# apache/arrow

Measured on AMD Instinct MI355X. Metric: filter_take_mrows_per_s, higher is better.
Workload: dtype int64; 1 GPU; Filter+Take int64[1000000000] + validity (10% null), boolean mask 10% true, FilterOptions::DROP; take indices = the mask's row numbers (monotonic; indices_nonzero: uint64 through CallFunction, GetTakeIndices: uint32 in the mirror), no boundscheck; inputs = splitmix64 streams of SURVEY.md 8(d) (seeds 1,2,3); rows=1000000000, selected_rows=99992053, parallelism=single-gpu

## Files before the change

### arrow_amd/_lib.py

```python
from __future__ import annotations

import ctypes as C
import os

_HERE = os.path.dirname(os.path.abspath(__file__))
LIB_PATH = os.path.join(_HERE, "libarrow_amd.so")

ARX_OK = 0
ARX_OUT_OF_MEMORY = -1
ARX_INVALID = -4
ARX_CAPACITY_ERROR = -6
ARX_INDEX_ERROR = -7
ARX_NOT_IMPLEMENTED = -10
ARX_DEVICE_ERROR = -100

ABI_VERSION = 5

FILTER_DROP, FILTER_EMIT_NULL = 0, 1
SORT_ASCENDING, SORT_DESCENDING = 0, 1
NULLS_AT_START, NULLS_AT_END = 0, 1


class ArrowAmdError(Exception):
    """Base class; subclasses mirror pyarrow.lib.ArrowInvalid & friends."""
# ... 61 lines not shown
        ("validity", C.c_void_p),
        ("offsets", C.c_void_p),
        ("data", C.c_void_p),
        ("offset", C.c_int64),
        ("length", C.c_int64),
        ("null_count", C.c_int64),
    ]


_p, _i64, _int, _u64, _u32, _sz = C.c_void_p, C.c_int64, C.c_int, C.c_uint64, C.c_uint32, C.c_size_t
_span = C.POINTER(ArxSpan)
_bspan = C.POINTER(ArxBinarySpan)

SIGNATURES = {
    "arx_last_error": (C.c_char_p, []),
    "arx_abi_version": (_int, []),
    "arx_device_count": (_int, []),
    "arx_set_option": (_int, [C.c_char_p, _i64]),
    "arx_get_option": (_int, [C.c_char_p, C.POINTER(_i64)]),
    "arx_get_counter": (_i64, [C.c_char_p]),
    "arx_filter_workspace_bytes": (_sz, [_i64]),
    "arx_filter_count": (_int, [_span, _int, _p, _sz, C.POINTER(_i64), _p]),
    "arx_filter_count_async": (_int, [_span, _int, _p, _sz, _p]),
    "arx_filter_count_nulls": (_int, [_span, _span, _int, _p, _sz, C.POINTER(_i64), C.POINTER(_i64), _p]),
    "arx_filter_exec": (_int, [_span, _int, _span, _int, _p, _i64, _p, _p, _p]),
    "arx_mask_to_indices": (_int, [_span, _int, _p, _i64, _int, _p, _p, _p]),
    "arx_filter_compact_form": (_int, [_int, _int, _int, _int, _i64, _i64]),
    "arx_take_workspace_bytes": (_sz, []),
    "arx_check_index_bounds": (_int, [_span, _int, _u64, _p, _sz, _p]),
    "arx_take": (_int, [_span, _int, _span, _int, _p, _p, _p, _p]),
    "arx_take_rows": (_int, [_span, _i64, _span, _int, _p, _p, _p, _p]),
    "arx_take_bits": (_int, [_span, _span, _int, _p, _p, _p, _p]),
    "arx_binary_take_workspace_bytes": (_sz, [_i64]),
    "arx_binary_take_offsets": (_int, [_bspan, _span, _int, _p, _sz, _p, _p, _p, C.POINTER(_i64), _p]),
    "arx_binary_take_data": (_int, [_bspan, _i64, _p, _sz, _p, _i64, _p, _p]),
    "arx_large_binary_take_workspace_bytes": (_sz, [_i64]),
    "arx_large_binary_take_offsets": (_int, [_bspan, _span, _int, _p, _sz, _p, _p, _p, C.POINTER(_i64), _p]),
    "arx_large_binary_take_data": (_int, [_bspan, _i64, _p, _sz, _p, _i64, _p, _p]),
    "arx_list_take_data": (_int, [_bspan, _int, _i64, _p, _sz, _p, _i64, _p, _p]),
    "arx_large_list_take_data": (_int, [_bspan, _int, _i64, _p, _sz, _p, _i64, _p, _p]),
    "arx_plain_byte_array_offsets": (_int, [_p, _sz, _i64, C.c_int32, _p]),
    "arx_rle_scan_runs": (_int, [_p, _sz, _int, _i64, _u32, _u64, _p, _i64, C.POINTER(_i64), C.POINTER(_i64)]),
    "arx_rle_decode_u32": (_int, [_p, _sz, _p, _i64, _int, _i64, _p, _p]),
    "arx_rle_decode_equals_bitmap": (_int, [_p, _sz, _p, _i64, _int, _i64, _u32, _p, _p]),
    "arx_expand_by_mask": (_int, [_p, _int, _span, _p, _p, _p]),
    "arx_rle_levels_to_bitmap": (_int, [_p, _p, _i64, _p, _p, _p, _p]),
    "arx_rle_scan_runs_equals": (_int, [_p, _sz, _int, _i64, _u32, _u32, _u64, _p, _i64, C.POINTER(_i64), C.POINTER(_i64)]),
    "arx_levels_to_list_workspace_bytes": (_sz, [_i64]),
# ... 203 lines not shown
```

### arrow_amd/csrc/plugin/common.inc

```

std::atomic<int64_t> g_gpu_calls{0};
std::atomic<int64_t> g_stock_calls{0};
std::atomic<int64_t> g_min_rows{1 << 16};
std::atomic<int64_t> g_min_rows_streaming{INT64_MAX};
std::atomic<int64_t> g_filter_morsel_rows{[] {
  const char* env = std::getenv("ARROW_AMD_FILTER_MORSEL_ROWS");
  return env != nullptr ? static_cast<int64_t>(std::strtoll(env, nullptr, 10)) : int64_t(1) << 20;
}()};

std::atomic<bool> g_parquet_pinned_staging{true};
std::atomic<bool> g_parquet_device_levels{true};
std::atomic<int> g_parquet_read_threads{4};
std::atomic<int64_t> g_parquet_read_part_bytes{int64_t(1) << 23};
std::atomic<bool> g_parquet_device_snappy{[] {
  const char* env = std::getenv("ARROW_AMD_PARQUET_DEVICE_SNAPPY");
  return env == nullptr || std::strtoll(env, nullptr, 10) != 0;
}()};
std::atomic<int64_t> g_parquet_device_snappy_pages{0};
std::atomic<bool> g_parquet_device_gzip{true};
std::atomic<int64_t> g_parquet_device_gzip_pages{0};
std::atomic<int64_t> g_parquet_copied_pages{0};

std::atomic<int64_t> g_aggregate_flush_rows{[] {
  const char* env = std::getenv("ARROW_AMD_AGGREGATE_FLUSH_ROWS");
// ... 68 lines not shown
    case ARX_CAPACITY_ERROR: return Status::CapacityError(msg);
    case ARX_INDEX_ERROR: return Status::IndexError(msg);
    case ARX_NOT_IMPLEMENTED: return Status::NotImplemented(msg);
    case ARX_OUT_OF_MEMORY: return Status::OutOfMemory(msg);
    default: return Status::UnknownError(msg);
  }
}

#define HIP_RETURN_NOT_OK(call)                                                        \
  do {                                                                                 \
    hipError_t e__ = (call);                                                           \
    if (e__ != hipSuccess)                                                             \
      return Status::IOError("HIP: ", hipGetErrorString(e__), " in " #call);           \
  } while (0)

thread_local hipStream_t t_stream = nullptr;

class DeviceScratch {
 public:
  ~DeviceScratch() {
    for (auto& s : slots_) {
      if (s.ptr) (void)hipFree(s.ptr);
    }
  }
  hipStream_t PeekStream() const { return stream_; }
  Status Stream(hipStream_t* out) {
    if (!stream_) {
      HIP_RETURN_NOT_OK(hipStreamCreateWithFlags(&stream_, hipStreamNonBlocking));
      t_stream = stream_;
    }
    *out = stream_;
    return Status::OK();
  }
  Status Get(int slot, size_t bytes, void** out) {
    if (slots_.size() <= static_cast<size_t>(slot)) slots_.resize(slot + 1);
    Slot& s = slots_[slot];
    bytes = (bytes + 255) & ~size_t(255);
    if (s.size < bytes) {
      if (s.ptr) HIP_RETURN_NOT_OK(hipFree(s.ptr));
      s.ptr = nullptr;
      s.size = 0;
      const size_t want = std::max<size_t>(bytes + bytes / 4, 1 << 20);
      HIP_RETURN_NOT_OK(hipMalloc(&s.ptr, want));
      s.size = want;
    }
    *out = s.ptr;
    return Status::OK();
  }

 private:
  struct Slot { void* ptr = nullptr; size_t size = 0; };
  std::vector<Slot> slots_;
  hipStream_t stream_ = nullptr;
};
thread_local DeviceScratch t_scratch;

class PinnedStaging {
 public:
  ~PinnedStaging() {
    if (ptr_) (void)hipHostFree(ptr_);
  }
  Status Reserve(size_t bytes, uint8_t** out) {
    if (size_ < bytes) {
      if (ptr_) HIP_RETURN_NOT_OK(hipHostFree(ptr_));
      ptr_ = nullptr;
      size_ = 0;
      const size_t want = std::max<size_t>(bytes + bytes / 4, size_t(1) << 20);
      HIP_RETURN_NOT_OK(hipHostMalloc(&ptr_, want, hipHostMallocDefault));
      size_ = want;
    }
    *out = static_cast<uint8_t*>(ptr_);
    return Status::OK();
  }
  void Trim(size_t keep_at_most) {
    if (size_ > keep_at_most && ptr_ != nullptr) {
      (void)hipHostFree(ptr_);
      ptr_ = nullptr;
      size_ = 0;
// ... 106 lines not shown
```

### arrow_amd/csrc/plugin/selection.inc

```
StockKernel g_stock_filter;

arrow::Result<std::unique_ptr<cp::KernelState>> FilterInit(cp::KernelContext* ctx,
                                                           const cp::KernelInitArgs& args) {
  auto state = std::make_unique<ShimState<cp::FilterOptions>>();
  if (g_stock_filter.init) {
    ARROW_ASSIGN_OR_RAISE(state->stock, g_stock_filter.init(ctx, args));
  }
  if (args.options != nullptr) {
    state->options = *static_cast<const cp::FilterOptions*>(args.options);
  }
  return state;
}

Status BooleanTakeOnDevice(const ArxSpan& dv, const ArxSpan& di, int tid, hipStream_t st, ArrayData* out_arr) {
  const int64_t m = di.length;
  const int64_t bytes = ((m + 63) / 64) * 8;
  const bool allocate_validity = dv.null_count != 0 || di.null_count != 0;
  out_arr->length = m;
  out_arr->buffers.resize(2);
  out_arr->buffers[0] = nullptr;
  ARROW_ASSIGN_OR_RAISE(out_arr->buffers[1], AllocDevice(bytes));
  void* d_valid = nullptr;
  void* d_counter = nullptr;
  if (allocate_validity) {
// ... 106 lines not shown
      if (allocate_validity) {
        ARROW_ASSIGN_OR_RAISE(out_arr->buffers[0], AllocDevice(((n + 63) / 64) * 8));
        d_valid = reinterpret_cast<void*>(out_arr->buffers[0]->mutable_address());
      }
      ARROW_RETURN_NOT_OK(FromArx(arx_filter_exec(&dv, w, &dm, null_sel, ws, n,
                                                  reinterpret_cast<void*>(out_arr->buffers[1]->mutable_address()),
                                                  d_valid, st)));
      int64_t selected = 0, set_bits = 0;
      HIP_RETURN_NOT_OK(hipMemcpyAsync(&selected, ws, 8, hipMemcpyDeviceToHost, st));
      if (allocate_validity) {
        void* cws = nullptr;
        ARROW_RETURN_NOT_OK(t_scratch.Get(kCounter, 64, &cws));
        ARROW_RETURN_NOT_OK(FromArx(arx_bitmap_popcount(d_valid, 0, n, cws, 64, &set_bits, st)));
      } else {
        HIP_RETURN_NOT_OK(hipStreamSynchronize(st));
      }
      out_arr->length = selected;
      out_arr->null_count = allocate_validity ? selected - set_bits : 0;
      static_cast<RocmBuffer*>(out_arr->buffers[1].get())->Shrink(selected * w);
      if (allocate_validity) static_cast<RocmBuffer*>(out_arr->buffers[0].get())->Shrink(((selected + 63) / 64) * 8);
      CountGpu(kFnFilter);
      return Status::OK();
    }
    int64_t out_len = 0, out_nulls = 0;
    if (allocate_validity) {
      ARROW_RETURN_NOT_OK(FromArx(arx_filter_count_nulls(&dv, &dm, null_sel, ws, ws_bytes, &out_len, &out_nulls, st)));
    } else {
      ARROW_RETURN_NOT_OK(FromArx(arx_filter_count(&dm, null_sel, ws, ws_bytes, &out_len, st)));
    }
    out_arr->length = out_len;
    out_arr->buffers.resize(2);
    ARROW_ASSIGN_OR_RAISE(out_arr->buffers[1], AllocDevice(out_len * w));
    out_arr->buffers[0] = nullptr;
    void* d_valid = nullptr;
    if (allocate_validity) {
      ARROW_ASSIGN_OR_RAISE(out_arr->buffers[0], AllocDevice(((out_len + 63) / 64) * 8));
      d_valid = reinterpret_cast<void*>(out_arr->buffers[0]->mutable_address());
    }
    ARROW_RETURN_NOT_OK(FromArx(arx_filter_exec(&dv, w, &dm, null_sel, ws, out_len,
                                                reinterpret_cast<void*>(out_arr->buffers[1]->mutable_address()),
                                                d_valid, st)));
    out_arr->null_count = allocate_validity ? out_nulls : 0;
    HIP_RETURN_NOT_OK(hipStreamSynchronize(st));
    CountGpu(kFnFilter);
    return Status::OK();
  }
  if (w == 0 || filter.type->id() != Type::BOOL || values.length < g_min_rows.load() ||
      !IsHost(values) || !IsHost(filter)) {
    return RunStock(kFnFilter, g_stock_filter, state->stock.get(), ctx, batch, out);
  }
  hipStream_t st;
  ARROW_RETURN_NOT_OK(t_scratch.Stream(&st));
  ArxSpan dv{}, dm{};
  ARROW_RETURN_NOT_OK(Upload(values, w, kValues, kValidity, st, &dv));
  ARROW_RETURN_NOT_OK(Upload(filter, 0, kArg2, kArg2Validity, st, &dm));
  const size_t ws_bytes = arx_filter_workspace_bytes(filter.length);
  void* ws = nullptr;
  ARROW_RETURN_NOT_OK(t_scratch.Get(kWs, ws_bytes, &ws));
  int64_t out_len = 0;
  ARROW_RETURN_NOT_OK(FromArx(arx_filter_count(&dm, null_sel, ws, ws_bytes, &out_len, st)));

  ArrayData* out_arr = out->array_data().get();
  const bool filter_null_count_is_zero = filter.null_count == 0;
  if (values.null_count == 0 && (null_sel == ARX_FILTER_DROP || filter_null_count_is_zero)) {
    out_arr->null_count = 0;
  } else {
// ... 326 lines not shown
```

### arrow_amd/csrc/plugin/vector_hash.inc

```
enum HashVectorKind { kHashUnique = 0, kHashValueCounts, kHashDictEncode };

struct DeviceHashState : public cp::KernelState {
  HashVectorKind kind = kHashUnique;
  std::unique_ptr<cp::KernelState> stock;
  bool used_stock = false, used_device = false;
  bool encode_nulls = false;
  std::shared_ptr<arrow::DataType> type;
  int width = 0;
  std::shared_ptr<Buffer> table_buf, counts_buf;
  void* table = nullptr;
  int64_t max_groups = 0, num_groups = 0, counts_cap = 0;
};

StockKernel g_stock_unique, g_stock_value_counts, g_stock_dict_encode;
cp::VectorKernel::FinalizeFunc g_stock_unique_finalize = nullptr, g_stock_value_counts_finalize = nullptr,
                               g_stock_dict_encode_finalize = nullptr;

template <HashVectorKind KIND>
const StockKernel& StockHashKernel() {
  return KIND == kHashUnique ? g_stock_unique : KIND == kHashValueCounts ? g_stock_value_counts : g_stock_dict_encode;
}

Status HashUniques(DeviceHashState* s, hipStream_t st, std::shared_ptr<Buffer>* values, std::shared_ptr<Buffer>* validity,
                   int64_t* null_count) {
// ... 293 lines not shown
  } else {
    const int num = NonZeroNumericTypeId(in.type->id());
    if (num < 0) return Status::NotImplemented("arrow_amd: indices_nonzero of device-resident ", in.type->ToString(), " arrays");
    static const int widths[10] = {1, 1, 2, 2, 4, 4, 8, 8, 4, 8};
    ARROW_ASSIGN_OR_RAISE(bits, AllocDevice(((n + 63) / 64) * 8 + 8));
    const uint64_t zero = 0;
    const uint8_t* base = static_cast<const uint8_t*>(dv.data) + dv.offset * widths[num];
    if (n > 0) {
      ARROW_RETURN_NOT_OK(FromArx(arx_compare_numeric(ARX_CMP_NOT_EQUAL, num, base, nullptr, nullptr, &zero, n,
                                                      reinterpret_cast<uint64_t*>(bits->mutable_address()), st)));
    }
    dm.data = reinterpret_cast<const void*>(bits->address());
    dm.offset = 0;
    if (dm.validity != nullptr && dv.offset != 0) {
      ARROW_ASSIGN_OR_RAISE(rebased, AllocDevice(((n + 63) / 64) * 8 + 8));
      ARROW_RETURN_NOT_OK(FromArx(arx_bitmap_copy(dv.validity, dv.offset, n, reinterpret_cast<void*>(rebased->mutable_address()), st)));
      dm.validity = reinterpret_cast<const void*>(rebased->address());
    }
  }
  const size_t ws_bytes = arx_filter_workspace_bytes(n);
  void* ws = nullptr;
  ARROW_RETURN_NOT_OK(t_scratch.Get(kWs, ws_bytes, &ws));
  int64_t cnt = 0;
  if (n > 0) ARROW_RETURN_NOT_OK(FromArx(arx_filter_count(&dm, ARX_FILTER_DROP, ws, ws_bytes, &cnt, st)));
  void* d_idx = nullptr;
  ARROW_RETURN_NOT_OK(t_scratch.Get(kArg2, static_cast<size_t>(cnt) * 4 + 64, &d_idx));
  ARROW_ASSIGN_OR_RAISE(auto out_values, AllocDevice(std::max<int64_t>(cnt, 1) * 8));
  bool direct = false;
  if (cnt > 0) {
    direct = arx_mask_to_indices(&dm, ARX_FILTER_DROP, ws, cnt, 8, reinterpret_cast<void*>(out_values->mutable_address()), nullptr, st) == ARX_OK;
  }
  if (cnt > 0 && !direct) {
    ARROW_RETURN_NOT_OK(FromArx(arx_mask_to_indices(&dm, ARX_FILTER_DROP, ws, cnt, 4, d_idx, nullptr, st)));
    ArxSpan di{nullptr, d_idx, 0, cnt, 0};
    void* flag = nullptr;
    ARROW_RETURN_NOT_OK(t_scratch.Get(kFlag, 64, &flag));
    ARROW_RETURN_NOT_OK(FromArx(arx_cast_numeric(&di, ARX_NUM_UINT32, ARX_NUM_UINT64, 1, 1, flag, 64,
                                                 reinterpret_cast<void*>(out_values->mutable_address()), st)));
  }
  HIP_RETURN_NOT_OK(hipStreamSynchronize(st));
  CountGpu(kFnFilter);
  out->value = ArrayData::Make(arrow::uint64(), cnt, {nullptr, std::move(out_values)}, 0);
  return Status::OK();
}

Status RegisterIndicesNonZero(cp::FunctionRegistry* reg) {
  ARROW_ASSIGN_OR_RAISE(auto fn, reg->GetFunction("indices_nonzero"));
// ... 72 lines not shown
```

### arrow_amd/csrc/selection.hip

```cpp
#include "arx_common.h"

#include <string.h>

#include <algorithm>
#include <type_traits>

namespace arx {

struct FilterWsHeader {
  int64_t total;
  int64_t ntiles;
  int64_t ngroups;
  int64_t length;
  int64_t valid;
  int64_t pad[3];
};
static_assert(sizeof(FilterWsHeader) == 64, "header is one 64-byte line");

struct FilterWsView {
  FilterWsHeader* hdr;
  int64_t* group_excl;
  int64_t* group_total;
  uint32_t* tile_counts;
  int64_t* group_valid;
};

static inline int64_t num_tiles(int64_t length) { return ceil_div(length, kTileRows); }
static inline int64_t num_groups(int64_t length) {
  return ceil_div(num_tiles(length), kTilesPerGroup);
}

static inline FilterWsView ws_view(void* ws, int64_t length) {
  FilterWsView v;
  const int64_t ng = num_groups(length);
  uint8_t* p = static_cast<uint8_t*>(ws);
  v.hdr = reinterpret_cast<FilterWsHeader*>(p);
  v.group_excl = reinterpret_cast<int64_t*>(p + 64);
  v.group_total = v.group_excl + ng;
  v.tile_counts = reinterpret_cast<uint32_t*>(v.group_total + ng);
  v.group_valid = reinterpret_cast<int64_t*>(v.tile_counts + ng * kTilesPerGroup);
  return v;
}

__device__ __forceinline__ uint64_t emit_word(const Bits& mask, const Bits& mvalid, int64_t w,
                                              bool emit_null, bool invert,
                                              uint64_t* mask_valid_out) {
  uint64_t m = load_word(mask, w);
  const uint64_t mv = load_word(mvalid, w);
  *mask_valid_out = mv;
  if (emit_null || invert) {
    const uint64_t in_range = load_word(Bits{nullptr, 0, mask.length, 0}, w);
    if (invert) m = ~m & in_range;
    if (emit_null) return (m | ~mv) & in_range;
  }
  return m & mv;
}

template <bool VALID>
__global__ __launch_bounds__(kBlock) void count_kernel(Bits mask, Bits mvalid, Bits vvalid, int emit_null,
                                                       int invert, int64_t ntiles,
                                                       uint32_t* tile_counts,
                                                       int64_t* group_total, int64_t* group_valid) {
  __shared__ uint32_t wave_sums[kWavesPerBlock];
  __shared__ uint32_t wave_valid[kWavesPerBlock];
  const int lane = lane_id();
  const int wave = threadIdx.x >> 6;
  const int64_t group = blockIdx.x;
  const int64_t t0 = group * kTilesPerGroup + wave * 16;
  uint32_t mine = 0;
  uint32_t kv = 0;
#pragma unroll 4
  for (int i = 0; i < 16; ++i) {
    const int64_t t = t0 + i;
    uint32_t k = 0;
    if (t < ntiles) {
      uint64_t mv;
      const uint64_t e = emit_word(mask, mvalid, t * 64 + lane, emit_null != 0, invert != 0, &mv);
      k = __popcll(e);
      if constexpr (VALID) kv += __popcll(e & mv & load_word(vvalid, t * 64 + lane));
    }
    const uint32_t s = wave_reduce_sum_u32(k);
    if (lane == i) mine = s;
  }
  if (lane < 16) tile_counts[t0 + lane] = mine;
  const uint32_t wsum = wave_reduce_sum_u32(lane < 16 ? mine : 0u);
  if (lane == 0) wave_sums[wave] = wsum;
  if constexpr (VALID) {
    const uint32_t vsum = wave_reduce_sum_u32(kv);
    if (lane == 0) wave_valid[wave] = vsum;
  }
  __syncthreads();
  if (threadIdx.x == 0) {
    int64_t s = 0, v = 0;
    for (int i = 0; i < kWavesPerBlock; ++i) {
      s += wave_sums[i];
      if constexpr (VALID) v += wave_valid[i];
    }
    group_total[group] = s;
    if constexpr (VALID) group_valid[group] = v;
  }
}

__global__ __launch_bounds__(1024) void scan_kernel(const int64_t* group_total, int64_t ngroups,
                                                    int64_t* group_excl, FilterWsHeader* hdr,
                                                    const int64_t* group_valid = nullptr) {
  __shared__ int64_t wave_tot[16];
  __shared__ int64_t carry_s;
  __shared__ unsigned long long valid_s;
  const int tid = threadIdx.x;
  const int lane = tid & 63;
  const int wave = tid >> 6;
  if (tid == 0) carry_s = 0;
  if (tid == 0) valid_s = 0;
  __syncthreads();
  if (group_valid != nullptr) {
    int64_t mine = 0;
    for (int64_t i = tid; i < ngroups; i += 1024) mine += group_valid[i];
#pragma unroll
    for (int d = 32; d >= 1; d >>= 1) mine += __shfl_xor(mine, d, 64);
    if (lane == 0 && mine != 0) atomicAdd(&valid_s, static_cast<unsigned long long>(mine));
    __syncthreads();
  }
  for (int64_t base = 0; base < ngroups; base += 1024) {
    const int64_t i = base + tid;
    const int64_t v = i < ngroups ? group_total[i] : 0;
    int64_t x = v;
#pragma unroll
    for (int d = 1; d < 64; d <<= 1) {
      const int64_t n = __shfl_up(x, d, 64);
      if (lane >= d) x += n;
    }
    if (lane == 63) wave_tot[wave] = x;
    __syncthreads();
    int64_t wave_prefix = 0;
    for (int k = 0; k < wave; ++k) wave_prefix += wave_tot[k];
    const int64_t carry = carry_s;
    if (i < ngroups) group_excl[i] = carry + wave_prefix + x - v;
    __syncthreads();
    if (tid == 1023) carry_s = carry + wave_prefix + x;
    __syncthreads();
  }
  if (tid == 0) {
    hdr->total = carry_s;
    hdr->valid = static_cast<int64_t>(valid_s);
  }
}

struct CompactArgs {
  const uint8_t* values;
  Bits mask;
  Bits mvalid;
  Bits vvalid;
  int64_t length;
  int64_t ntiles;
  const uint32_t* tile_counts;
  const int64_t* group_excl;
  uint8_t* out_data;
  uint64_t* out_validity;
  int emit_null;
  int invert;
  int values_aligned16;
};

constexpr int kFlushBytes = 2048;

template <int RING>
struct __attribute__((aligned(16))) CompactLds {
  uint8_t ring[kWavesPerBlock][RING];
  uint64_t vbits[kWavesPerBlock][72];
};

template <int W>
struct ElemT;
template <> struct ElemT<1> { using type = uint8_t; };
template <> struct ElemT<2> { using type = uint16_t; };
template <> struct ElemT<4> { using type = uint32_t; };
template <> struct ElemT<8> { using type = uint64_t; };
template <> struct ElemT<16> { using type = uint4; };
struct Elem32 { uint4 lo, hi; };
template <> struct ElemT<32> { using type = Elem32; };

template <int W>
__device__ __forceinline__ typename ElemT<W>::type zero_elem() {
  if constexpr (W == 32) {
// ... 387 lines not shown
  const uint32_t p = incl - k;
  const int total = static_cast<int>(__shfl(incl, 63, 64));
  if (total == 0) return;

  const int64_t grp = t >> 6;
  const int tin = static_cast<int>(t & 63);
  const uint32_t cprev = lane < tin ? a.tile_counts[grp * kTilesPerGroup + lane] : 0u;
  const int64_t off = a.group_excl[grp] + wave_reduce_sum_u32(cprev);

  uint16_t* sel = lds.sel[wave];
  const bool want_validity = a.out_validity != nullptr;
  if (want_validity) lds.vs[wave][lane] = load_word(a.vvalid, w) & mv;
  if constexpr (EMIT) lds.zw[wave][lane] = Ew & ~mv;

  const E* __restrict__ values = IOTA ? nullptr : reinterpret_cast<const E*>(a.values) + t * kTileRows;
  E* __restrict__ out = reinterpret_cast<E*>(a.out_data);
  const int head = static_cast<int>(off & 63);
  const int nsteps = (head + total + 63) >> 6;
  const int64_t word0 = off >> 6;
  constexpr int kStepsPerWindow = kSparseWindow / 64;

  uint64_t m = Ew;
  uint32_t rk = p;
  for (int step0 = 0; step0 < nsteps; step0 += kStepsPerWindow) {
    const int win_lo = step0 * 64 - head;
    const int win_hi = win_lo + kSparseWindow;
    while (m != 0 && static_cast<int>(rk) < win_hi) {
      const int bpos = __ffsll(static_cast<unsigned long long>(m)) - 1;
      m &= m - 1;
      sel[static_cast<int>(rk) - win_lo] = static_cast<uint16_t>(lane * 64 + bpos);
      ++rk;
    }
    wave_lds_sync();
    const int step_end = (step0 + kStepsPerWindow) < nsteps ? (step0 + kStepsPerWindow) : nsteps;
    const int first_listed = win_lo < 0 ? 0 : win_lo;
    for (int i0 = step0; i0 < step_end; i0 += U) {
      int s[U];
      bool act[U];
      int r[U];
      E v[U];
#pragma unroll
      for (int u = 0; u < U; ++u) {
        s[u] = (i0 + u) * 64 + lane - head;
        act[u] = s[u] >= 0 && s[u] < total && (i0 + u) < step_end;
        r[u] = sel[(act[u] ? s[u] : first_listed) - win_lo];
      }
#pragma unroll
      for (int u = 0; u < U; ++u) {
        if constexpr (IOTA) {
          if constexpr (W <= 8) v[u] = static_cast<E>(t * kTileRows + r[u]);
        } else {
          v[u] = sel_load<W>(values + r[u], (kSelNt & 1) != 0);
        }
      }
#pragma unroll
      for (int u = 0; u < U; ++u) {
        if ((i0 + u) >= step_end) break;
        E e = v[u];
        if constexpr (EMIT) {
          if ((lds.zw[wave][r[u] >> 6] >> (r[u] & 63)) & 1ull) e = zero_elem<W>();
        }
        if (act[u]) sel_store<W>(out + off + s[u], e);
        if (want_validity) {
          const bool vbit = act[u] && ((lds.vs[wave][r[u] >> 6] >> (r[u] & 63)) & 1ull);
          const uint64_t bal = __ballot(vbit);
          const uint64_t owned = __ballot(act[u]);
          if (lane == 0) {
            uint64_t* dst = a.out_validity + word0 + i0 + u;
            if (owned == ~uint64_t(0)) {
              *dst = bal;
            } else if (bal != 0) {
              atomicOr(reinterpret_cast<unsigned long long*>(dst), static_cast<unsigned long long>(bal));
            }
          }
        }
      }
    }
    wave_lds_sync();
  }
}

template <int W>
__global__ __launch_bounds__(kBlock) void expand_kernel(CompactArgs a) {
  using E = typename ElemT<W>::type;
  __shared__ uint64_t words[kWavesPerBlock][64];
  __shared__ uint32_t before[kWavesPerBlock][64];
  const int lane = lane_id();
  const int wave = __builtin_amdgcn_readfirstlane(threadIdx.x >> 6);
  const int64_t t = static_cast<int64_t>(blockIdx.x) * kWavesPerBlock + wave;
  if (t >= a.ntiles) return;
  uint64_t mv;
  const uint64_t mw = emit_word(a.mask, a.mvalid, t * 64 + lane, false, false, &mv);
  const uint32_t k = __popcll(mw);
  const uint32_t incl = wave_inclusive_scan_u32(k);
  words[wave][lane] = mw;
  before[wave][lane] = incl - k;
  const int64_t grp = t >> 6;
  const int tin = static_cast<int>(t & 63);
  const uint32_t cprev = lane < tin ? a.tile_counts[grp * kTilesPerGroup + lane] : 0u;
  const int64_t off = a.group_excl[grp] + wave_reduce_sum_u32(cprev);
  wave_lds_sync();
// ... 357 lines not shown
    set_error("filter mask is NULL");
    return ARX_INVALID;
  }
  if (mask->length < 0 || mask->offset < 0) {
    set_error("negative length/offset");
    return ARX_INVALID;
  }
  if (mask->length > 0 && mask->data == nullptr) {
    set_error("filter mask has no data buffer");
    return ARX_INVALID;
  }
  if (null_selection != ARX_FILTER_DROP && null_selection != ARX_FILTER_EMIT_NULL) {
    set_error("bad null_selection %d", null_selection);
    return ARX_INVALID;
  }
  return ARX_OK;
}

static inline const void* effective_validity(const ArxSpan* s) {
  return (s->null_count != 0) ? s->validity : nullptr;
}

static int launch_count(const ArxSpan* mask, int null_selection, void* ws, size_t ws_bytes,
                        hipStream_t st, int invert = 0, const ArxSpan* values = nullptr) {
  const int rc = check_mask(mask, null_selection);
  if (rc != ARX_OK) return rc;
  const size_t need = arx_filter_workspace_bytes(mask->length);
  if (ws == nullptr || ws_bytes < need) {
    set_error("filter workspace too small: %zu < %zu", ws_bytes, need);
    return ARX_INVALID;
  }
  if ((reinterpret_cast<uint64_t>(ws) & 63) != 0) {
    set_error("filter workspace must be 64-byte aligned");
    return ARX_INVALID;
  }
  FilterWsView v = ws_view(ws, mask->length);
  const int64_t nt = num_tiles(mask->length);
  const int64_t ng = num_groups(mask->length);
  FilterWsHeader h{};
  h.total = 0;
  h.ntiles = nt;
  h.ngroups = ng;
  h.length = mask->length;
  ARX_HIP(hipMemcpyAsync(v.hdr, &h, sizeof(h), hipMemcpyHostToDevice, st));
  if (mask->length == 0) return ARX_OK;
  const Bits mb = make_bits(mask->data, mask->offset, mask->length);
  const Bits mvb = make_bits(effective_validity(mask), mask->offset, mask->length);
  if (values != nullptr) {
    const Bits vvb = make_bits(effective_validity(values), values->offset, mask->length);
    hipLaunchKernelGGL((count_kernel<true>), dim3(static_cast<unsigned>(ng)), dim3(kBlock), 0, st, mb, mvb, vvb,
                       null_selection, invert, nt, v.tile_counts, v.group_total, v.group_valid);
    ARX_CHECK_LAUNCH("count_kernel");
    hipLaunchKernelGGL(scan_kernel, dim3(1), dim3(1024), 0, st, v.group_total, ng, v.group_excl, v.hdr,
                       static_cast<const int64_t*>(v.group_valid));
  } else {
    hipLaunchKernelGGL((count_kernel<false>), dim3(static_cast<unsigned>(ng)), dim3(kBlock), 0, st, mb, mvb, mvb,
                       null_selection, invert, nt, v.tile_counts, v.group_total, static_cast<int64_t*>(nullptr));
    ARX_CHECK_LAUNCH("count_kernel");
    hipLaunchKernelGGL(scan_kernel, dim3(1), dim3(1024), 0, st, v.group_total, ng, v.group_excl, v.hdr,
                       static_cast<const int64_t*>(nullptr));
  }
  ARX_CHECK_LAUNCH("scan_kernel");
  return ARX_OK;
}

static Knob<int> g_filter_batch{4};
static Knob<int> g_filter_pipe{1};
static Knob<int> g_filter_sparse{-1};
static const KnobRow kSelectionKnobs[] = {
    {"filter_batch", g_filter_batch, knob_snap_down<1, 4>},
    {"filter_pipe", g_filter_pipe, knob_bool},
    {"filter_sparse", g_filter_sparse, knob_tri},
};
KnobTable selection_knobs() { return knob_table(kSelectionKnobs); }

template <int W, bool IOTA, bool EMIT, bool ALIGNED>
static void launch_compact_e(const CompactArgs& a, unsigned grid, hipStream_t st) {
  constexpr int kIters = kTileRows / (kWave * (16 / W));
  constexpr int kBig = kIters >= 8 ? 4 : 2;
  if (ALIGNED && g_filter_batch >= 4 && g_filter_pipe) {
    hipLaunchKernelGGL((compact_kernel<W, IOTA, EMIT, ALIGNED, kBig, true>), dim3(grid),
                       dim3(kBlock), 0, st, a);
  } else {
// ... 133 lines not shown
  a.mvalid = make_bits(nullptr, 0, length);
  a.vvalid = make_bits(nullptr, 0, length);
  a.length = length;
  a.ntiles = num_tiles(length);
  a.tile_counts = v.tile_counts;
  a.group_excl = v.group_excl;
  a.out_data = reinterpret_cast<uint8_t*>(out);
  a.out_validity = nullptr;
  a.emit_null = 0;
  a.invert = invert ? 1 : 0;
  a.values_aligned16 = 1;
  return launch_compact(true, 4, a, st);
}

}

using namespace arx;

extern "C" {

size_t arx_filter_workspace_bytes(int64_t length) {
  if (length < 0) length = 0;
  const int64_t ng = num_groups(length);
  return static_cast<size_t>(64 + ng * 16 + ng * kTilesPerGroup * 4 + ng * 8 + 64);
}

int arx_filter_count_async(const ArxSpan* mask, int null_selection, void* ws, size_t ws_bytes,
                           void* stream) {
  return launch_count(mask, null_selection, ws, ws_bytes, as_stream(stream));
}

int arx_filter_count_nulls(const ArxSpan* values, const ArxSpan* mask, int null_selection, void* ws, size_t ws_bytes,
                           int64_t* out_length, int64_t* out_null_count, void* stream) {
  if (out_length == nullptr || out_null_count == nullptr || values == nullptr) {
    set_error("values / out_length / out_null_count is NULL");
    return ARX_INVALID;
  }
  if (mask != nullptr && values->length != mask->length) {
    set_error("filter values and mask differ in length (%lld vs %lld)", static_cast<long long>(values->length),
              static_cast<long long>(mask->length));
    return ARX_INVALID;
  }
  hipStream_t st = as_stream(stream);
  const int rc = launch_count(mask, null_selection, ws, ws_bytes, st, 0, values);
  if (rc != ARX_OK) return rc;
  int64_t hdr[5] = {0, 0, 0, 0, 0};
  ARX_HIP(hipMemcpyAsync(hdr, ws, sizeof(hdr), hipMemcpyDeviceToHost, st));
  ARX_HIP(hipStreamSynchronize(st));
  *out_length = hdr[0];
  *out_null_count = mask->length == 0 ? 0 : hdr[0] - hdr[4];
  return ARX_OK;
}

int arx_filter_count(const ArxSpan* mask, int null_selection, void* ws, size_t ws_bytes,
                     int64_t* out_length, void* stream) {
  if (out_length == nullptr) {
    set_error("out_length is NULL");
    return ARX_INVALID;
  }
  hipStream_t st = as_stream(stream);
  const int rc = launch_count(mask, null_selection, ws, ws_bytes, st);
  if (rc != ARX_OK) return rc;
  int64_t total = 0;
  ARX_HIP(hipMemcpyAsync(&total, ws, sizeof(int64_t), hipMemcpyDeviceToHost, st));
  ARX_HIP(hipStreamSynchronize(st));
  *out_length = total;
  return ARX_OK;
}

int arx_filter_exec(const ArxSpan* values, int byte_width, const ArxSpan* mask, int null_selection,
                    const void* ws, int64_t out_length, void* out_data, void* out_validity,
                    void* stream) {
  int rc = check_mask(mask, null_selection);
  if (rc != ARX_OK) return rc;
  if (values == nullptr || ws == nullptr) {
    set_error("values/ws is NULL");
    return ARX_INVALID;
  }
  if (values->length != mask->length) {
    set_error("Array arguments must all be the same length (values %lld vs filter %lld)",
              static_cast<long long>(values->length), static_cast<long long>(mask->length));
    return ARX_INVALID;
  }
  if (mask->length == 0) return ARX_OK;
  if (values->data == nullptr || out_data == nullptr) {
    set_error("values/out data buffer is NULL");
    return ARX_INVALID;
  }
  hipStream_t st = as_stream(stream);
  FilterWsView v = ws_view(const_cast<void*>(ws), mask->length);
  CompactArgs a{};
  a.values = static_cast<const uint8_t*>(values->data) + values->offset * byte_width;
  a.mask = make_bits(mask->data, mask->offset, mask->length);
  a.mvalid = make_bits(effective_validity(mask), mask->offset, mask->length);
  a.vvalid = make_bits(effective_validity(values), values->offset, values->length);
  a.length = mask->length;
  a.ntiles = num_tiles(mask->length);
  a.tile_counts = v.tile_counts;
  a.group_excl = v.group_excl;
  a.out_data = static_cast<uint8_t*>(out_data);
  a.out_validity = static_cast<uint64_t*>(out_validity);
  a.emit_null = null_selection == ARX_FILTER_EMIT_NULL && a.mvalid.base != nullptr;
  a.values_aligned16 = (reinterpret_cast<uint64_t>(a.values) & 15) == 0;
  if ((reinterpret_cast<uint64_t>(out_data) % byte_width) != 0) {
    set_error("out_data is not aligned to the element width");
    return ARX_INVALID;
  }
  rc = zero_out_validity(out_validity, out_length, st);
  if (rc != ARX_OK) return rc;
  return launch_compact(false, byte_width, a, st, out_length);
}

int arx_expand_by_mask(const void* dense, int byte_width, const ArxSpan* mask, const void* ws, void* out_data,
                       void* stream) {
  int rc = check_mask(mask, ARX_FILTER_DROP);
  if (rc != ARX_OK) return rc;
  if (ws == nullptr) {
    set_error("ws is NULL (run arx_filter_count on the mask first)");
    return ARX_INVALID;
  }
  if (mask->length == 0) return ARX_OK;
  if (out_data == nullptr || (reinterpret_cast<uint64_t>(out_data) % byte_width) != 0 ||
      (dense != nullptr && (reinterpret_cast<uint64_t>(dense) % byte_width) != 0)) {
    set_error("expand: NULL or misaligned buffer");
    return ARX_INVALID;
  }
  FilterWsView v = ws_view(const_cast<void*>(ws), mask->length);
  CompactArgs a{};
  a.values = static_cast<const uint8_t*>(dense);
  a.mask = make_bits(mask->data, mask->offset, mask->length);
  a.mvalid = make_bits(effective_validity(mask), mask->offset, mask->length);
  a.length = mask->length;
  a.ntiles = num_tiles(mask->length);
// ... 423 lines not shown
```

### include/arrow_amd.h

```cpp
#ifndef ARROW_AMD_H_
#define ARROW_AMD_H_

#include <stddef.h>
#include <stdint.h>

#ifdef __cplusplus
extern "C" {
#endif

#define ARX_ABI_VERSION 5

typedef enum ArxStatus {
  ARX_OK = 0,
  ARX_OUT_OF_MEMORY = -1,
  ARX_INVALID = -4,
  ARX_CAPACITY_ERROR = -6,
  ARX_INDEX_ERROR = -7,
  ARX_NOT_IMPLEMENTED = -10,
  ARX_DEVICE_ERROR = -100
} ArxStatus;

enum { ARX_FILTER_DROP = 0, ARX_FILTER_EMIT_NULL = 1 };
enum { ARX_SORT_ASCENDING = 0, ARX_SORT_DESCENDING = 1 };
enum { ARX_NULLS_AT_START = 0, ARX_NULLS_AT_END = 1 };
// ... 10 lines not shown
  int64_t length;
  int64_t null_count;
} ArxSpan;

const char* arx_last_error(void);
int arx_abi_version(void);
int arx_device_count(void);
int arx_set_option(const char* name, int64_t value);
int arx_get_option(const char* name, int64_t* out_value);
int64_t arx_get_counter(const char* name);


size_t arx_filter_workspace_bytes(int64_t length);

int arx_filter_count(const ArxSpan* mask, int null_selection, void* ws, size_t ws_bytes,
                     int64_t* out_length, void* stream);

int arx_filter_count_nulls(const ArxSpan* values, const ArxSpan* mask, int null_selection, void* ws, size_t ws_bytes,
                           int64_t* out_length, int64_t* out_null_count, void* stream);

int arx_filter_count_async(const ArxSpan* mask, int null_selection, void* ws,
                           size_t ws_bytes, void* stream);

int arx_filter_exec(const ArxSpan* values, int byte_width, const ArxSpan* mask,
                    int null_selection, const void* ws, int64_t out_length, void* out_data,
                    void* out_validity, void* stream);

int arx_mask_to_indices(const ArxSpan* mask, int null_selection, const void* ws,
                        int64_t out_length, int index_width, void* out_indices,
                        void* out_validity, void* stream);

enum { ARX_COMPACT_GATHER = 0, ARX_COMPACT_SWEEP_PIPELINED = 1, ARX_COMPACT_SWEEP_PLAIN = 2, ARX_COMPACT_SWEEP_UNALIGNED = 3 };

int arx_filter_compact_form(int row_numbers, int byte_width, int values_aligned16, int invert,
                            int64_t length, int64_t out_length);

size_t arx_take_workspace_bytes(void);

int arx_check_index_bounds(const ArxSpan* indices, int index_type, uint64_t upper_limit,
                           void* ws, size_t ws_bytes, void* stream);

int arx_take(const ArxSpan* values, int byte_width, const ArxSpan* indices, int index_type,
             void* out_data, void* out_validity, int64_t* valid_count, void* stream);

int arx_take_rows(const ArxSpan* values, int64_t row_bytes, const ArxSpan* indices, int index_type, void* out_data,
                  void* out_validity, int64_t* valid_count, void* stream);

int arx_take_columns(const ArxSpan* columns, const int32_t* byte_widths, int num_columns, const ArxSpan* indices,
                     int index_type, void* const* out_data, void* const* out_validity, int64_t* valid_counts,
// ... 604 lines not shown
```

Measured before the change: 291,900 Mrows/s.

## Count output validity inside gather compaction and trim count-kernel overheads

When the filter path needs output validity and the gather compaction form applies, the count pass now computes only the selected-row count. The output null count is accumulated inside the compaction kernel via sharded atomics, so the value validity bitmap is not read a second time during counting. The count kernel also batches all 16 tile loads up front, packs two 16-bit popcounts per reduction, and takes an aligned fast path. The header write moves into the scan kernel, which writes its total to a pinned host word and drops a host-to-device memcpy. The cost is an extra tiny reduction kernel, atomics in compaction, and more API surface.

```diff
diff --git a/arrow_amd/_lib.py b/arrow_amd/_lib.py
--- a/arrow_amd/_lib.py
+++ b/arrow_amd/_lib.py
@@ -107,8 +107,10 @@
     "arx_filter_workspace_bytes": (_sz, [_i64]),
     "arx_filter_count": (_int, [_span, _int, _p, _sz, C.POINTER(_i64), _p]),
     "arx_filter_count_async": (_int, [_span, _int, _p, _sz, _p]),
+    "arx_filter_count_to": (_int, [_span, _int, _p, _sz, _p, _p]),
     "arx_filter_count_nulls": (_int, [_span, _span, _int, _p, _sz, C.POINTER(_i64), C.POINTER(_i64), _p]),
     "arx_filter_exec": (_int, [_span, _int, _span, _int, _p, _i64, _p, _p, _p]),
+    "arx_filter_exec_nulls": (_int, [_span, _int, _span, _int, _p, _i64, _p, _p, _p, _p]),
     "arx_mask_to_indices": (_int, [_span, _int, _p, _i64, _int, _p, _p, _p]),
     "arx_filter_compact_form": (_int, [_int, _int, _int, _int, _i64, _i64]),
     "arx_take_workspace_bytes": (_sz, []),
diff --git a/arrow_amd/csrc/plugin/common.inc b/arrow_amd/csrc/plugin/common.inc
--- a/arrow_amd/csrc/plugin/common.inc
+++ b/arrow_amd/csrc/plugin/common.inc
@@ -114,6 +114,7 @@
     for (auto& s : slots_) {
       if (s.ptr) (void)hipFree(s.ptr);
     }
+    if (words_) (void)hipHostFree(words_);
   }
   hipStream_t PeekStream() const { return stream_; }
   Status Stream(hipStream_t* out) {
@@ -139,13 +140,28 @@
     *out = s.ptr;
     return Status::OK();
   }
+  Status ResultWords(int64_t** out) {
+    if (!words_) HIP_RETURN_NOT_OK(hipHostMalloc(reinterpret_cast<void**>(&words_), 64, hipHostMallocDefault));
+    *out = words_;
+    return Status::OK();
+  }
 
  private:
   struct Slot { void* ptr = nullptr; size_t size = 0; };
   std::vector<Slot> slots_;
+  int64_t* words_ = nullptr;
   hipStream_t stream_ = nullptr;
 };
 thread_local DeviceScratch t_scratch;
+
+Status CountMaskRows(const ArxSpan& dm, int null_sel, void* ws, size_t ws_bytes, hipStream_t st, int64_t* out_len) {
+  int64_t* words = nullptr;
+  ARROW_RETURN_NOT_OK(t_scratch.ResultWords(&words));
+  ARROW_RETURN_NOT_OK(FromArx(arx_filter_count_to(&dm, null_sel, ws, ws_bytes, &words[0], st)));
+  HIP_RETURN_NOT_OK(hipStreamSynchronize(st));
+  *out_len = words[0];
+  return Status::OK();
+}
 
 class PinnedStaging {
  public:
diff --git a/arrow_amd/csrc/plugin/selection.inc b/arrow_amd/csrc/plugin/selection.inc
--- a/arrow_amd/csrc/plugin/selection.inc
+++ b/arrow_amd/csrc/plugin/selection.inc
@@ -152,8 +152,15 @@
       CountGpu(kFnFilter);
       return Status::OK();
     }
+    const bool count_in_compaction =
+        allocate_validity && w >= 8 && arx_filter_compact_form(0, w, 1, 0, filter.length, -1) == ARX_COMPACT_GATHER;
     int64_t out_len = 0, out_nulls = 0;
-    if (allocate_validity) {
+    int64_t* valid_word = nullptr;
+    if (count_in_compaction) {
+      ARROW_RETURN_NOT_OK(t_scratch.ResultWords(&valid_word));
+      valid_word += 1;
+      ARROW_RETURN_NOT_OK(CountMaskRows(dm, null_sel, ws, ws_bytes, st, &out_len));
+    } else if (allocate_validity) {
       ARROW_RETURN_NOT_OK(FromArx(arx_filter_count_nulls(&dv, &dm, null_sel, ws, ws_bytes, &out_len, &out_nulls, st)));
     } else {
       ARROW_RETURN_NOT_OK(FromArx(arx_filter_count(&dm, null_sel, ws, ws_bytes, &out_len, st)));
@@ -167,11 +174,19 @@
       ARROW_ASSIGN_OR_RAISE(out_arr->buffers[0], AllocDevice(((out_len + 63) / 64) * 8));
       d_valid = reinterpret_cast<void*>(out_arr->buffers[0]->mutable_address());
     }
-    ARROW_RETURN_NOT_OK(FromArx(arx_filter_exec(&dv, w, &dm, null_sel, ws, out_len,
-                                                reinterpret_cast<void*>(out_arr->buffers[1]->mutable_address()),
-                                                d_valid, st)));
+    const bool counted = count_in_compaction && out_len > 0;
+    if (counted) {
+      ARROW_RETURN_NOT_OK(FromArx(arx_filter_exec_nulls(&dv, w, &dm, null_sel, ws, out_len,
+                                                        reinterpret_cast<void*>(out_arr->buffers[1]->mutable_address()),
+                                                        d_valid, valid_word, st)));
+    } else {
+      ARROW_RETURN_NOT_OK(FromArx(arx_filter_exec(&dv, w, &dm, null_sel, ws, out_len,
+                                                  reinterpret_cast<void*>(out_arr->buffers[1]->mutable_address()),
+                                                  d_valid, st)));
+    }
+    HIP_RETURN_NOT_OK(hipStreamSynchronize(st));
+    if (counted) out_nulls = out_len - *valid_word;
     out_arr->null_count = allocate_validity ? out_nulls : 0;
-    HIP_RETURN_NOT_OK(hipStreamSynchronize(st));
     CountGpu(kFnFilter);
     return Status::OK();
   }
diff --git a/arrow_amd/csrc/plugin/vector_hash.inc b/arrow_amd/csrc/plugin/vector_hash.inc
--- a/arrow_amd/csrc/plugin/vector_hash.inc
+++ b/arrow_amd/csrc/plugin/vector_hash.inc
@@ -339,7 +339,7 @@
   void* ws = nullptr;
   ARROW_RETURN_NOT_OK(t_scratch.Get(kWs, ws_bytes, &ws));
   int64_t cnt = 0;
-  if (n > 0) ARROW_RETURN_NOT_OK(FromArx(arx_filter_count(&dm, ARX_FILTER_DROP, ws, ws_bytes, &cnt, st)));
+  if (n > 0) ARROW_RETURN_NOT_OK(CountMaskRows(dm, ARX_FILTER_DROP, ws, ws_bytes, st, &cnt));
   void* d_idx = nullptr;
   ARROW_RETURN_NOT_OK(t_scratch.Get(kArg2, static_cast<size_t>(cnt) * 4 + 64, &d_idx));
   ARROW_ASSIGN_OR_RAISE(auto out_values, AllocDevice(std::max<int64_t>(cnt, 1) * 8));
diff --git a/arrow_amd/csrc/selection.hip b/arrow_amd/csrc/selection.hip
--- a/arrow_amd/csrc/selection.hip
+++ b/arrow_amd/csrc/selection.hip
@@ -23,7 +23,11 @@
   int64_t* group_total;
   uint32_t* tile_counts;
   int64_t* group_valid;
+  unsigned long long* valid_shards;
 };
+
+constexpr int kValidShards = 64;
+constexpr int kValidShardStride = 32;
 
 static inline int64_t num_tiles(int64_t length) { return ceil_div(length, kTileRows); }
 static inline int64_t num_groups(int64_t length) {
@@ -39,6 +43,7 @@
   v.group_total = v.group_excl + ng;
   v.tile_counts = reinterpret_cast<uint32_t*>(v.group_total + ng);
   v.group_valid = reinterpret_cast<int64_t*>(v.tile_counts + ng * kTilesPerGroup);
+  v.valid_shards = reinterpret_cast<unsigned long long*>(v.group_valid + ng);
   return v;
 }
 
@@ -56,34 +61,78 @@
   return m & mv;
 }
 
-template <bool VALID>
+template <bool ALIGNED>
+__device__ __forceinline__ uint64_t count_load_word(const Bits& b, int64_t w) {
+  if constexpr (ALIGNED) {
+    const int64_t last = b.nphys - 1;
+    const uint64_t v = b.base[w < last ? w : last];
+    const int64_t remain = b.length - (w << 6);
+    const uint64_t m = remain >= 64 ? ~uint64_t(0) : (remain <= 0 ? uint64_t(0) : ((uint64_t(1) << remain) - 1));
+    return v & m;
+  } else {
+    return load_word_nb(b, w);
+  }
+}
+
+template <bool VALID, bool ALIGNED>
 __global__ __launch_bounds__(kBlock) void count_kernel(Bits mask, Bits mvalid, Bits vvalid, int emit_null,
                                                        int invert, int64_t ntiles,
                                                        uint32_t* tile_counts,
                                                        int64_t* group_total, int64_t* group_valid) {
   __shared__ uint32_t wave_sums[kWavesPerBlock];
   __shared__ uint32_t wave_valid[kWavesPerBlock];
+  constexpr int kT = 16;
   const int lane = lane_id();
   const int wave = threadIdx.x >> 6;
   const int64_t group = blockIdx.x;
-  const int64_t t0 = group * kTilesPerGroup + wave * 16;
+  const int64_t t0 = group * kTilesPerGroup + wave * kT;
+  (void)ntiles;
+  const Bits in_range = Bits{nullptr, 0, mask.length, 0};
+  uint64_t m[kT], mv[kT], vv[kT];
+#pragma unroll
+  for (int i = 0; i < kT; ++i) m[i] = count_load_word<ALIGNED>(mask, (t0 + i) * 64 + lane);
+  if (mvalid.base != nullptr) {
+#pragma unroll
+    for (int i = 0; i < kT; ++i) mv[i] = count_load_word<ALIGNED>(mvalid, (t0 + i) * 64 + lane);
+  } else {
+#pragma unroll
+    for (int i = 0; i < kT; ++i) mv[i] = load_word(in_range, (t0 + i) * 64 + lane);
+  }
+  if constexpr (VALID) {
+    if (vvalid.base != nullptr) {
+#pragma unroll
+      for (int i = 0; i < kT; ++i) vv[i] = count_load_word<ALIGNED>(vvalid, (t0 + i) * 64 + lane);
+    } else {
+#pragma unroll
+      for (int i = 0; i < kT; ++i) vv[i] = ~uint64_t(0);
+    }
+  }
+  uint32_t pk[kT / 2];
+  uint32_t kv = 0;
+#pragma unroll
+  for (int i = 0; i < kT; ++i) {
+    uint64_t e = m[i];
+    if (emit_null != 0 || invert != 0) {
+      const uint64_t inr = load_word(in_range, (t0 + i) * 64 + lane);
+      if (invert != 0) e = ~e & inr;
+      e = emit_null != 0 ? ((e | ~mv[i]) & inr) : (e & mv[i]);
+    } else {
+      e &= mv[i];
+    }
+    const uint32_t k = __popcll(e);
+    if constexpr (VALID) kv += __popcll(e & mv[i] & vv[i]);
+    if ((i & 1) == 0) pk[i >> 1] = k;
+    else pk[i >> 1] |= k << 16;
+  }
   uint32_t mine = 0;
-  uint32_t kv = 0;
-#pragma unroll 4
-  for (int i = 0; i < 16; ++i) {
-    const int64_t t = t0 + i;
-    uint32_t k = 0;
-    if (t < ntiles) {
-      uint64_t mv;
-      const uint64_t e = emit_word(mask, mvalid, t * 64 + lane, emit_null != 0, invert != 0, &mv);
-      k = __popcll(e);
-      if constexpr (VALID) kv += __popcll(e & mv & load_word(vvalid, t * 64 + lane));
-    }
-    const uint32_t s = wave_reduce_sum_u32(k);
-    if (lane == i) mine = s;
-  }
-  if (lane < 16) tile_counts[t0 + lane] = mine;
-  const uint32_t wsum = wave_reduce_sum_u32(lane < 16 ? mine : 0u);
+#pragma unroll
+  for (int j = 0; j < kT / 2; ++j) {
+    const uint32_t s = wave_reduce_sum_u32(pk[j]);
+    if (lane == 2 * j) mine = s & 0xFFFFu;
+    if (lane == 2 * j + 1) mine = s >> 16;
+  }
+  if (lane < kT) tile_counts[t0 + lane] = mine;
+  const uint32_t wsum = wave_reduce_sum_u32(lane < kT ? mine : 0u);
   if (lane == 0) wave_sums[wave] = wsum;
   if constexpr (VALID) {
     const uint32_t vsum = wave_reduce_sum_u32(kv);
@@ -103,7 +152,8 @@
 
 __global__ __launch_bounds__(1024) void scan_kernel(const int64_t* group_total, int64_t ngroups,
                                                     int64_t* group_excl, FilterWsHeader* hdr,
-                                                    const int64_t* group_valid = nullptr) {
+                                                    const int64_t* group_valid, int64_t ntiles, int64_t length,
+                                                    unsigned long long* valid_shards, int64_t* total_out) {
   __shared__ int64_t wave_tot[16];
   __shared__ int64_t carry_s;
   __shared__ unsigned long long valid_s;
@@ -140,10 +190,23 @@
     if (tid == 1023) carry_s = carry + wave_prefix + x;
     __syncthreads();
   }
+  if (tid < kValidShards) valid_shards[tid * kValidShardStride] = 0;
   if (tid == 0) {
     hdr->total = carry_s;
+    if (total_out != nullptr) *total_out = carry_s;
+    hdr->ntiles = ntiles;
+    hdr->ngroups = ngroups;
+    hdr->length = length;
     hdr->valid = static_cast<int64_t>(valid_s);
-  }
+    hdr->pad[0] = hdr->pad[1] = hdr->pad[2] = 0;
+  }
+}
+
+__global__ __launch_bounds__(kWave) void valid_total_kernel(const unsigned long long* valid_shards, int64_t* out) {
+  const int lane = lane_id();
+  static_assert(kValidShards == kWave, "one shard per lane");
+  const uint64_t s = wave_reduce_sum_u64(valid_shards[lane * kValidShardStride]);
+  if (lane == 0) *out = static_cast<int64_t>(s);
 }
 
 struct CompactArgs {
@@ -160,6 +223,7 @@
   int emit_null;
   int invert;
   int values_aligned16;
+  unsigned long long* valid_shards;
 };
 
 constexpr int kFlushBytes = 2048;
@@ -593,6 +657,7 @@
 
   uint64_t m = Ew;
   uint32_t rk = p;
+  uint32_t nvalid = 0;
   for (int step0 = 0; step0 < nsteps; step0 += kStepsPerWindow) {
     const int win_lo = step0 * 64 - head;
     const int win_hi = win_lo + kSparseWindow;
@@ -636,6 +701,7 @@
           const bool vbit = act[u] && ((lds.vs[wave][r[u] >> 6] >> (r[u] & 63)) & 1ull);
           const uint64_t bal = __ballot(vbit);
           const uint64_t owned = __ballot(act[u]);
+          nvalid += __popcll(bal);
           if (lane == 0) {
             uint64_t* dst = a.out_validity + word0 + i0 + u;
             if (owned == ~uint64_t(0)) {
@@ -648,6 +714,9 @@
       }
     }
     wave_lds_sync();
+  }
+  if (want_validity && a.valid_shards != nullptr && lane == 0 && nvalid != 0) {
+    atomicAdd(&a.valid_shards[(blockIdx.x & (kValidShards - 1)) * kValidShardStride], static_cast<unsigned long long>(nvalid));
   }
 }
 
@@ -1051,7 +1120,8 @@
 }
 
 static int launch_count(const ArxSpan* mask, int null_selection, void* ws, size_t ws_bytes,
-                        hipStream_t st, int invert = 0, const ArxSpan* values = nullptr) {
+                        hipStream_t st, int invert = 0, const ArxSpan* values = nullptr,
+                        int64_t* total_out = nullptr) {
   const int rc = check_mask(mask, null_selection);
   if (rc != ARX_OK) return rc;
   const size_t need = arx_filter_workspace_bytes(mask->length);
@@ -1066,28 +1136,37 @@
   FilterWsView v = ws_view(ws, mask->length);
   const int64_t nt = num_tiles(mask->length);
   const int64_t ng = num_groups(mask->length);
-  FilterWsHeader h{};
-  h.total = 0;
-  h.ntiles = nt;
-  h.ngroups = ng;
-  h.length = mask->length;
-  ARX_HIP(hipMemcpyAsync(v.hdr, &h, sizeof(h), hipMemcpyHostToDevice, st));
-  if (mask->length == 0) return ARX_OK;
+  if (mask->length == 0) {
+    hipLaunchKernelGGL(scan_kernel, dim3(1), dim3(1024), 0, st, v.group_total, ng, v.group_excl, v.hdr,
+                       static_cast<const int64_t*>(nullptr), nt, mask->length, v.valid_shards, total_out);
+    ARX_CHECK_LAUNCH("scan_kernel");
+    return ARX_OK;
+  }
   const Bits mb = make_bits(mask->data, mask->offset, mask->length);
   const Bits mvb = make_bits(effective_validity(mask), mask->offset, mask->length);
   if (values != nullptr) {
     const Bits vvb = make_bits(effective_validity(values), values->offset, mask->length);
-    hipLaunchKernelGGL((count_kernel<true>), dim3(static_cast<unsigned>(ng)), dim3(kBlock), 0, st, mb, mvb, vvb,
-                       null_selection, invert, nt, v.tile_counts, v.group_total, v.group_valid);
+    if (mb.shift == 0 && mvb.shift == 0 && vvb.shift == 0) {
+      hipLaunchKernelGGL((count_kernel<true, true>), dim3(static_cast<unsigned>(ng)), dim3(kBlock), 0, st, mb, mvb, vvb,
+                         null_selection, invert, nt, v.tile_counts, v.group_total, v.group_valid);
+    } else {
+      hipLaunchKernelGGL((count_kernel<true, false>), dim3(static_cast<unsigned>(ng)), dim3(kBlock), 0, st, mb, mvb, vvb,
+                         null_selection, invert, nt, v.tile_counts, v.group_total, v.group_valid);
+    }
     ARX_CHECK_LAUNCH("count_kernel");
     hipLaunchKernelGGL(scan_kernel, dim3(1), dim3(1024), 0, st, v.group_total, ng, v.group_excl, v.hdr,
-                       static_cast<const int64_t*>(v.group_valid));
+                       static_cast<const int64_t*>(v.group_valid), nt, mask->length, v.valid_shards, total_out);
   } else {
-    hipLaunchKernelGGL((count_kernel<false>), dim3(static_cast<unsigned>(ng)), dim3(kBlock), 0, st, mb, mvb, mvb,
-                       null_selection, invert, nt, v.tile_counts, v.group_total, static_cast<int64_t*>(nullptr));
+    if (mb.shift == 0 && mvb.shift == 0) {
+      hipLaunchKernelGGL((count_kernel<false, true>), dim3(static_cast<unsigned>(ng)), dim3(kBlock), 0, st, mb, mvb, mvb,
+                         null_selection, invert, nt, v.tile_counts, v.group_total, static_cast<int64_t*>(nullptr));
+    } else {
+      hipLaunchKernelGGL((count_kernel<false, false>), dim3(static_cast<unsigned>(ng)), dim3(kBlock), 0, st, mb, mvb, mvb,
+                         null_selection, invert, nt, v.tile_counts, v.group_total, static_cast<int64_t*>(nullptr));
+    }
     ARX_CHECK_LAUNCH("count_kernel");
     hipLaunchKernelGGL(scan_kernel, dim3(1), dim3(1024), 0, st, v.group_total, ng, v.group_excl, v.hdr,
-                       static_cast<const int64_t*>(nullptr));
+                       static_cast<const int64_t*>(nullptr), nt, mask->length, v.valid_shards, total_out);
   }
   ARX_CHECK_LAUNCH("scan_kernel");
   return ARX_OK;
@@ -1267,12 +1346,21 @@
 size_t arx_filter_workspace_bytes(int64_t length) {
   if (length < 0) length = 0;
   const int64_t ng = num_groups(length);
-  return static_cast<size_t>(64 + ng * 16 + ng * kTilesPerGroup * 4 + ng * 8 + 64);
+  return static_cast<size_t>(64 + ng * 16 + ng * kTilesPerGroup * 4 + ng * 8 + kValidShards * kValidShardStride * 8 + 64);
 }
 
 int arx_filter_count_async(const ArxSpan* mask, int null_selection, void* ws, size_t ws_bytes,
                            void* stream) {
   return launch_count(mask, null_selection, ws, ws_bytes, as_stream(stream));
+}
+
+int arx_filter_count_to(const ArxSpan* mask, int null_selection, void* ws, size_t ws_bytes, int64_t* out_length,
+                        void* stream) {
+  if (out_length == nullptr) {
+    set_error("out_length is NULL");
+    return ARX_INVALID;
+  }
+  return launch_count(mask, null_selection, ws, ws_bytes, as_stream(stream), 0, nullptr, out_length);
 }
 
 int arx_filter_count_nulls(const ArxSpan* values, const ArxSpan* mask, int null_selection, void* ws, size_t ws_bytes,
@@ -1313,9 +1401,9 @@
   return ARX_OK;
 }
 
-int arx_filter_exec(const ArxSpan* values, int byte_width, const ArxSpan* mask, int null_selection,
-                    const void* ws, int64_t out_length, void* out_data, void* out_validity,
-                    void* stream) {
+static int filter_exec(const ArxSpan* values, int byte_width, const ArxSpan* mask, int null_selection,
+                       const void* ws, int64_t out_length, void* out_data, void* out_validity,
+                       bool counted, int64_t* out_valid_count, void* stream) {
   int rc = check_mask(mask, null_selection);
   if (rc != ARX_OK) return rc;
   if (values == nullptr || ws == nullptr) {
@@ -1327,7 +1415,14 @@
               static_cast<long long>(values->length), static_cast<long long>(mask->length));
     return ARX_INVALID;
   }
-  if (mask->length == 0) return ARX_OK;
+  if (mask->length == 0) {
+    if (counted && out_valid_count != nullptr) {
+      hipLaunchKernelGGL(valid_total_kernel, dim3(1), dim3(kWave), 0, as_stream(stream),
+                         ws_view(const_cast<void*>(ws), 0).valid_shards, out_valid_count);
+      ARX_CHECK_LAUNCH("valid_total_kernel");
+    }
+    return ARX_OK;
+  }
   if (values->data == nullptr || out_data == nullptr) {
     set_error("values/out data buffer is NULL");
     return ARX_INVALID;
@@ -1351,9 +1446,39 @@
     set_error("out_data is not aligned to the element width");
     return ARX_INVALID;
   }
+  if (counted) {
+    if (out_validity == nullptr || out_valid_count == nullptr) {
+      set_error("arx_filter_exec_nulls needs out_validity and out_valid_count");
+      return ARX_INVALID;
+    }
+    if (compact_form(false, byte_width, a.values_aligned16 != 0, false, a.length, out_length) != ARX_COMPACT_GATHER) {
+      set_error("arx_filter_exec_nulls: only the gather form counts (byte width %d, filter_sparse %d)", byte_width,
+                static_cast<int>(g_filter_sparse));
+      return ARX_NOT_IMPLEMENTED;
+    }
+    a.valid_shards = v.valid_shards;
+  }
   rc = zero_out_validity(out_validity, out_length, st);
   if (rc != ARX_OK) return rc;
-  return launch_compact(false, byte_width, a, st, out_length);
+  rc = launch_compact(false, byte_width, a, st, out_length);
+  if (rc != ARX_OK || !counted) return rc;
+  hipLaunchKernelGGL(valid_total_kernel, dim3(1), dim3(kWave), 0, st, v.valid_shards, out_valid_count);
+  ARX_CHECK_LAUNCH("valid_total_kernel");
+  return ARX_OK;
+}
+
+int arx_filter_exec(const ArxSpan* values, int byte_width, const ArxSpan* mask, int null_selection,
+                    const void* ws, int64_t out_length, void* out_data, void* out_validity,
+                    void* stream) {
+  return filter_exec(values, byte_width, mask, null_selection, ws, out_length, out_data, out_validity, false, nullptr,
+                     stream);
+}
+
+int arx_filter_exec_nulls(const ArxSpan* values, int byte_width, const ArxSpan* mask, int null_selection,
+                          const void* ws, int64_t out_length, void* out_data, void* out_validity,
+                          int64_t* out_valid_count, void* stream) {
+  return filter_exec(values, byte_width, mask, null_selection, ws, out_length, out_data, out_validity, true,
+                     out_valid_count, stream);
 }
 
 int arx_expand_by_mask(const void* dense, int byte_width, const ArxSpan* mask, const void* ws, void* out_data,
diff --git a/include/arrow_amd.h b/include/arrow_amd.h
--- a/include/arrow_amd.h
+++ b/include/arrow_amd.h
@@ -56,9 +56,16 @@
 int arx_filter_count_async(const ArxSpan* mask, int null_selection, void* ws,
                            size_t ws_bytes, void* stream);
 
+int arx_filter_count_to(const ArxSpan* mask, int null_selection, void* ws, size_t ws_bytes,
+                        int64_t* out_length, void* stream);
+
 int arx_filter_exec(const ArxSpan* values, int byte_width, const ArxSpan* mask,
                     int null_selection, const void* ws, int64_t out_length, void* out_data,
                     void* out_validity, void* stream);
+
+int arx_filter_exec_nulls(const ArxSpan* values, int byte_width, const ArxSpan* mask,
+                          int null_selection, const void* ws, int64_t out_length, void* out_data,
+                          void* out_validity, int64_t* out_valid_count, void* stream);
 
 int arx_mask_to_indices(const ArxSpan* mask, int null_selection, const void* ws,
                         int64_t out_length, int index_width, void* out_indices,
```

Result: faster. 297,700 Mrows/s (median of 6 runs) (+2.0%).
